# silvery107/rl-mpc-locomotion

Measured on AMD Instinct MI355X. Metric: MPC control steps/sec (whole node) @ horizon=10, 4096 robots; max |GRF| err vs OSQP, higher is better.
Workload: dtype f64; 1 GPU; config 2: 4096 robots/GPU x 1 GPU(s), Aliengo, trot, horizon=10, flat terrain (BASELINE configs[1]); one controller.run(dof_states, body_states, commands) -> torques call per step with EVERY robot due for its MPC update: state estimator, leg kinematics, gait / foot placement, compute_contact_forces (QP build + solve), swing / stance commands, leg-torque map a22 = SURVEY.md 8(d)'s unit of work; war; seam=ctrl, robots_per_gpu=4096, robots_total=4096, horizon=10, parallelism=robot-sharded x1

## Files before the change

rl-mpc-locomotion_amd/csrc/mpc_core.h:

```cpp
#pragma once

#include <math.h>
#include <stdint.h>

#if defined(__HIPCC__)
#define MPC_HD __host__ __device__ __forceinline__
#else
#define MPC_HD inline
#endif
#if defined(__HIP_DEVICE_COMPILE__)
#define MPC_LAUNDER(x) asm volatile("" : "+v"(x))
#define MPC_SCHED_FENCE() __builtin_amdgcn_sched_barrier(0)
#define MPC_LDS_STORE64(p, v) (*(volatile __attribute__((address_space(3))) double *)(p) = (v))
#define MPC_LDS_LOAD64(p) (*(const volatile __attribute__((address_space(3))) double *)(p))
typedef double mpc_double2 __attribute__((ext_vector_type(2)));
#define MPC_LDS_LOAD128(p, lo, hi) do { const mpc_double2 v2_ = *(const volatile __attribute__((address_space(3))) mpc_double2 *)(p); (lo) = v2_.x; (hi) = v2_.y; } while (0)
#define MPC_GST(p, v) __hip_atomic_store((p), (v), __ATOMIC_RELAXED, __HIP_MEMORY_SCOPE_AGENT)
#define MPC_GLD(p) __hip_atomic_load((p), __ATOMIC_RELAXED, __HIP_MEMORY_SCOPE_AGENT)
#define MPC_WAIT_LOADS() __builtin_amdgcn_s_waitcnt(0x0F70)
#define MPC_WAIT_LDS() __builtin_amdgcn_s_waitcnt(0xC07F)
#else
#define MPC_WAIT_LOADS() ((void)0)
#define MPC_WAIT_LDS() ((void)0)
#define MPC_GST(p, v) (*(p) = (v))
// ... 34 lines not shown
#define MPC_CLOCK() ((long long)__builtin_readcyclecounter())
#else
#define MPC_CLOCK() (0LL)
#endif

namespace mpc {

#if defined(__HIPCC__)
typedef _Float16 mpc_half;
MPC_HD double half_to_double(mpc_half v) { return (double)v; }
#else
typedef unsigned short mpc_half;
inline double half_to_double(mpc_half b) {
  const int sgn = b >> 15, ex = (b >> 10) & 31, man = b & 1023;
  double v;
  if (ex == 0) v = ldexp((double)man, -24);
  else if (ex == 31) v = man ? NAN : INFINITY;
  else v = ldexp((double)(man | 1024), ex - 25);
  return sgn ? -v : v;
}
#endif

constexpr double kRho0 = 0.1, kSigma = 1e-6, kAlphaRelax = 1.6;
constexpr double kEpsAbs = 1e-3, kEpsRel = 1e-3;
constexpr int kMaxIter = 4000, kCheck = 25;
constexpr double kRhoMin = 1e-6, kRhoMax = 1e6, kRhoEqOverIneq = 1e3, kRhoTol = 1e-4;
constexpr int kScalingIters = 10;
constexpr double kMinScaling = 1e-4, kMaxScaling = 1e4, kAdaptTol = 5.0;
constexpr double kInfty = 1e30, kDelta = 1e-6;
constexpr int kPolishRefine = 3;
constexpr double kGravity = 9.8, kMaxScale = 10.0, kMinScale = 0.1;

constexpr int kStSolved = 1, kStSolvedInaccurate = 2, kStPrimInfInaccurate = 3, kStDualInfInaccurate = 4, kStMaxIter = -2, kStPrimInf = -3, kStDualInf = -4,
              kStNonCvx = -7, kStUnsolved = -10;

constexpr int kAsPos[9] = {0, 2, 3, 5, 7, 8, 10, 11, 14};

template <int H>
struct Cfg {
  static constexpr int N = 12 * H, M = 20 * H, NF = 4 * H;
  static constexpr int TS = 6;
  static constexpr int G = N / TS;
  static constexpr int MT = G * (G + 1) / 2;
  static constexpr int NT = H > 16 ? MPC_NT_H20 : (H > 12 ? MPC_NT_H16 : 1);
  static constexpr int MTH = (MT + NT - 1) / NT;
  static constexpr int TE = TS * TS;
  static constexpr int T0 = (((MTH > N ? MTH : N) + 63) / 64) * 64;
  static constexpr int T = T0 < 128 ? 128 : T0;
  static constexpr int MR = (M + T - 1) / T;
  static constexpr int IN_LEN = 56 + 4 * H;
  static_assert(T <= 1024, "workgroup too large");
  static constexpr int NP = N + 2;
  static constexpr bool kQInLds = H > 12;
#ifdef MPC_PIN_MASK
  static constexpr int kPinMask = MPC_PIN_MASK;
#else
  static constexpr int kPinMask = H > 16 ? 3 : 17;
#endif
  static constexpr int QP_Q = 0, QP_BND = N, QP_CONE = N + 3 * NF, QP_B6 = QP_CONE + 16, QP_TH1 = QP_B6 + 72,
                       QP_TH2 = QP_TH1 + 36, QP_LEN = QP_TH2 + 8;
  static constexpr int SC_D = 0, SC_E = N, SC_QS = N + M, SC_C = 2 * N + M, SC_JOB = SC_C + 2, SC_LEN = SC_C + 4;
  static MPC_HD double scaled_cone_entry(const double *qp, const double *sc, int f, int k) {
    const int pos = kAsPos[k];
    return (qp[QP_CONE + pos] * sc[SC_E + 5 * f + pos / 3]) * sc[SC_D + 3 * f + pos % 3];
  }
  static MPC_HD double scaled_cone_entry(double a, double e, double d) { return (a * e) * d; }
  static constexpr int XQP_L = N, XQP_U = N + M, XQP_CONE = N + 2 * M, XQP_LEN = XQP_CONE + 16 + 72 + 36 + 8;
  static constexpr int XSC_AS = 2 * N + M, XSC_LS = XSC_AS + 15 * NF, XSC_US = XSC_LS + M, XSC_C = XSC_US + M, XSC_LEN = XSC_C + 4;
  static constexpr int NW = 6 * H, GW = H, MTW = H * (H + 1) / 2;
  static constexpr int FOOT0 = MPC_FOOT0(H, MTW);
  static constexpr int TWMIN = FOOT0 + NF > MTW ? FOOT0 + NF : MTW;
  static constexpr int TW = (((TWMIN > NW ? TWMIN : NW) + 63) / 64) * 64;
  static constexpr int NPW = NW + 2;
};

constexpr int IN_W = 0, IN_POS = 13, IN_VEL = 16, IN_RPY = 19, IN_NRM = 22, IN_ANG = 25, IN_CONTACT = 28;
template <int H> constexpr int in_foot() { return 28 + 4 * H; }
template <int H> constexpr int in_fric() { return 40 + 4 * H; }
template <int H> constexpr int in_dpos() { return 44 + 4 * H; }
template <int H> constexpr int in_dvel() { return 47 + 4 * H; }
template <int H> constexpr int in_drpy() { return 50 + 4 * H; }
template <int H> constexpr int in_dang() { return 53 + 4 * H; }

template <int H> constexpr int state_len() { return 2 * Cfg<H>::N + 2 * Cfg<H>::M + 2; }

constexpr int kInfoLen = 8;
constexpr int kProfLen = 16;

struct RobotModel {
  double mass, inv_mass, inv_inertia[9], dt, alpha;
};

#define MPC_V alignas(16) double
template <int H>
struct ScaleShared {
  using C = Cfg<H>;
  MPC_V q[C::kQInLds ? C::N : 2];
  MPC_V qs[C::N]; MPC_V As[C::NF * 15];
  MPC_V D[C::N]; MPC_V E[C::M];
  double c, cinv, ctmp;
  int first;
  MPC_V xt[C::N];
  MPC_V cone[16];
  MPC_V dt_[C::N]; MPC_V et_[C::M];
  MPC_V part[C::NP * C::G];
};
template <int H>
struct AsmShared {
  using C = Cfg<H>;
  MPC_V in[C::IN_LEN];
  static constexpr int XK = 13 * H > 74 ? 13 * H : 74;
  MPC_V x0[13]; MPC_V xref[13 * H]; MPC_V sdiff[XK]; MPC_V xk[XK];
  MPC_V a_dt[169]; MPC_V b_dt[156]; MPC_V a_exp[169]; MPC_V b_exp[156];
  MPC_V wanb[H * 156];
  MPC_V B6[72]; MPC_V th1[36]; MPC_V th2[8];
};
template <int H>
struct PrepShared {
  union {
    AsmShared<H> as;
    ScaleShared<H> sc;
  };
  MPC_V u12[288];
};
#undef MPC_V

template <int H>
struct Thread {
  using C = Cfg<H>;
  int tid;
  int ti[C::NT], tj[C::NT];
  bool mact[C::NT], dia[C::NT];
  double Mx[C::NT * C::TE];
  static constexpr int VPL = (C::N + 63) / 64;
  double rm[VPL];
  double red[2];
  MPC_HD void init(int id) {
    tid = id;
    for (int u = 0; u < C::NT; ++u) {
      const int tile = id + u * C::MTH;
      mact[u] = id < C::MTH && tile < C::MT;
      int r = 0;
      while ((r + 1) * (r + 2) / 2 <= tile) ++r;
      ti[u] = r; tj[u] = tile - r * (r + 1) / 2; dia[u] = ti[u] == tj[u];
    }
  }
};

struct TileView {
  int ti, tj, index;
  bool dia;
  double *Mx;
};

MPC_HD double limit_scaling(double v) {
  v = v < kMinScaling ? 1.0 : v;
  return v > kMaxScaling ? kMaxScaling : v;
}
MPC_HD double dmax(double a, double b) { return a > b ? a : b; }
MPC_HD double dmin(double a, double b) { return a < b ? a : b; }
MPC_HD double raw_max(double a, double b) {
#if defined(__HIP_DEVICE_COMPILE__)
  double r;
  asm("v_max_f64 %0, %1, %2" : "=v"(r) : "v"(a), "v"(b));
  return r;
#else
  return fmax(a, b);
#endif
}
MPC_HD double raw_min(double a, double b) {
#if defined(__HIP_DEVICE_COMPILE__)
  double r;
  asm("v_min_f64 %0, %1, %2" : "=v"(r) : "v"(a), "v"(b));
  return r;
#else
  return fmin(a, b);
#endif
}
MPC_HD double clampd(double v, double lo, double hi) { return raw_min(raw_max(v, lo), hi); }

MPC_HD int mpc_ffs64(unsigned long long v) {
#if defined(__HIP_DEVICE_COMPILE__)
  return __ffsll((long long)v) - 1;
#else
  return __builtin_ctzll(v);
#endif
}

MPC_HD unsigned long long dbits(double v) {
  union { double d; unsigned long long u; } c;
  c.d = v;
  return c.u;
}
MPC_HD double bitsd(unsigned long long u) {
  union { double d; unsigned long long u; } c;
  c.u = u;
  return c.d;
}

#ifndef MPC_PROFILE_SUB
#define MPC_PROFILE_SUB 0
#endif
#define MPC_SUBLAP(sec, k) do { if (MPC_PROFILE_SUB == (sec)) lap(k); } while (0)

template <int H, class Exec>
struct Assembler {
  using C = Cfg<H>;
  using Th = Thread<H>;
  static constexpr int N = C::N, M = C::M, NF = C::NF, T = C::T, TS = C::TS, TE = C::TE;

  Exec &ex;
  AsmShared<H> &s;
  const RobotModel &mdl;
  const float *in;
  const double *in64;
  const mpc_half *in16;
  double *u12;
  double *qp;
  long long *prof;
  long long tc[16] = {0, 0, 0, 0, 0, 0, 0, 0, 0, 0, 0, 0, 0, 0, 0, 0};
  long long tlast = 0;
#ifndef MPC_SECTION_PROFILE
  MPC_HD void lap(int) {}
#else
  MPC_HD void lap(int k) { const long long now = MPC_CLOCK(); tc[k] += now - tlast; tlast = now; }
#endif

  static MPC_HD double mat3e(const double *a, const double *b, int e) {
    const int i = e / 3, j = e - 3 * i;
    return a[3 * i] * b[j] + a[3 * i + 1] * b[3 + j] + a[3 * i + 2] * b[6 + j];
  }

  MPC_HD double in_at(int i) const { return in64 ? in64[i] : (in16 ? half_to_double(in16[i]) : (double)in[i]); }
  MPC_HD void run() {
    tlast = MPC_CLOCK();
    double *const trig = s.xk, *const fw = s.xk + 43, *const iw = s.xk + 64;
    double *const iib = s.sdiff + 53;
    static_assert(AsmShared<H>::XK >= 73, "xk / sdiff too small for the set-up scratch");
    ex.par([&](Th &t) {
      for (int i = t.tid; i < C::IN_LEN; i += T) s.in[i] = in_at(i);
      for (int i = t.tid; i < 169; i += T) s.a_dt[i] = 0;
      for (int i = t.tid; i < 156; i += T) s.b_dt[i] = 0;
      for (int i = t.tid; i < 72; i += T) { qp[C::QP_B6 + i] = 0; s.B6[i] = 0; }
      if (t.tid >= 64 && t.tid < 67) {
        const int k = t.tid - 64;
        const double ang = in_at(IN_RPY + k);
        trig[2 * k] = cos(ang); trig[2 * k + 1] = sin(ang);
        if (k == 1) trig[6] = tan(ang);
      } else if (t.tid >= 96 && t.tid < 105) {
        iib[t.tid - 96] = mdl.inv_inertia[t.tid - 96];
      }
    });
    MPC_SUBLAP(4, 9);
    ex.par([&](Th &t) {
      if (t.tid == 0) {
        const double cr = trig[0], sr = trig[1], cp = trig[2], sp = trig[3], cy = trig[4], sy = trig[5];
        const double rx[9] = {1.0, 0.0, 0.0, 0.0, cr, -sr, 0.0, sr, cr};
        const double ry[9] = {cp, 0.0, sp, 0.0, 1.0, 0.0, -sp, 0.0, cp};
        const double rz[9] = {cy, -sy, 0.0, sy, cy, 0.0, 0.0, 0.0, 1.0};
        double m1[9], m2[9], rxyz[9], rzyx[9], t2[9], ib[9];
#pragma unroll
        for (int e = 0; e < 9; ++e) { m1[e] = mat3e(rx, ry, e); m2[e] = mat3e(rz, ry, e); ib[e] = iib[e]; }
#pragma unroll
        for (int e = 0; e < 9; ++e) { rxyz[e] = mat3e(m1, rz, e); rzyx[e] = mat3e(m2, rx, e); }
        const double *fb = s.in + in_foot<H>();
#pragma unroll
        for (int i = 0; i < 4; ++i)
#pragma unroll
          for (int r = 0; r < 3; ++r) fw[3 * i + r] = rxyz[3 * r] * fb[3 * i] + rxyz[3 * r + 1] * fb[3 * i + 1] + rxyz[3 * r + 2] * fb[3 * i + 2];
#pragma unroll
        for (int e = 0; e < 9; ++e) t2[e] = mat3e(rzyx, ib, e);
#pragma unroll
        for (int i = 0; i < 3; ++i)
#pragma unroll
          for (int j = 0; j < 3; ++j) iw[3 * i + j] = t2[3 * i] * rzyx[3 * j] + t2[3 * i + 1] * rzyx[3 * j + 1] + t2[3 * i + 2] * rzyx[3 * j + 2];
      }
      if (t.tid >= 32 && t.tid < 45) {
        const int i = t.tid - 32;
        s.x0[i] = i < 3 ? s.in[IN_RPY + i] : i < 6 ? s.in[IN_POS + i - 3] : i < 9 ? s.in[IN_ANG + i - 6] : i < 12 ? s.in[IN_VEL + i - 9] : -kGravity;
      }
      for (int f = t.tid; f < NF; f += T) {
        const double cst = s.in[IN_CONTACT + f];
        const double fzmax = mdl.mass * kGravity * kMaxScale, fzmin = mdl.mass * kGravity * kMinScale;
        const double mu0 = s.in[in_fric<H>()];
        qp[C::QP_BND + 3 * f] = dmax(fzmin * cst, -kInfty);
        qp[C::QP_BND + 3 * f + 1] = dmin((mu0 + 1) * fzmax * cst, kInfty);
        qp[C::QP_BND + 3 * f + 2] = dmin(fzmax * cst, kInfty);
      }
      for (int k = t.tid; k < 13 * H; k += T) {
        const int i = k / 13, r = k - 13 * i;
        const double tt = mdl.dt * (i + 1);
        const int drpy = in_drpy<H>(), dvel = in_dvel<H>(), dang = in_dang<H>(), dpos = in_dpos<H>();
        const int bi = r < 2 ? drpy + r : r == 2 ? IN_RPY + 2 : r < 5 ? IN_POS + r - 3 : r == 5 ? dpos + 2 : r < 9 ? dang + r - 6 : dvel + (r < 11 ? r - 9 : 0);
        const int si = r == 2 ? dang + 2 : dvel + (r == 4 ? 1 : 0);
        const double base = s.in[bi], slope = s.in[si];
        const double v = (r == 2 || r == 3 || r == 4) ? tt * slope + base : base;
        s.xref[k] = r == 11 ? 0.0 : r == 12 ? -kGravity : v;
      }
    });
    MPC_SUBLAP(4, 12);
    ex.par([&](Th &t) {
      const double dt = mdl.dt;
      if (t.tid < 36) {
        const int i = t.tid / 9, e = t.tid - 9 * i, r = e / 3, c = e - 3 * r;
        const double *v = fw + 3 * i;
        double acc = 0;
        for (int k = 0; k < 3; ++k) {
          const double sk = (k == c) ? 0.0 : (((c - k + 3) % 3 == 1) ? -v[3 - k - c] : v[3 - k - c]);
          const double term = iw[3 * r + k] * sk;
          acc = k == 0 ? term : acc + term;
        }
        s.b_dt[(6 + r) * 12 + 3 * i + c] = acc * dt;
        qp[C::QP_B6 + r * 12 + 3 * i + c] = acc;
        s.B6[r * 12 + 3 * i + c] = acc;
      } else if (t.tid < 48) {
        const int k = t.tid - 36, i = k / 3, r = k - 3 * i;
        s.b_dt[(9 + r) * 12 + 3 * i + r] = mdl.inv_mass * dt;
        qp[C::QP_B6 + (3 + r) * 12 + 3 * i + r] = mdl.inv_mass;
        s.B6[(3 + r) * 12 + 3 * i + r] = mdl.inv_mass;
      } else if (t.tid < 57) {
        const int e = t.tid - 48, r = e / 3, c = e - 3 * r;
        const double cp = trig[2], cy = trig[4], sy = trig[5], tp = trig[6];
        const double num = c == 0 ? cy : sy;
        double val;
        if (c == 2) val = r == 2 ? 1.0 : 0.0;
        else if (r == 0) val = num / cp;
        else if (r == 1) val = c == 0 ? -sy : cy;
        else val = num * tp;
        s.a_dt[r * 13 + 6 + c] = val * dt;
      } else if (t.tid < 60) {
        const int r = t.tid - 57;
        s.a_dt[(3 + r) * 13 + 9 + r] = dt;
        s.a_dt[(9 + r) * 13 + 12] = s.in[IN_NRM + r] * dt;
      } else if (t.tid == 60) {
        const double *fr = s.in + in_fric<H>();
        const double cb[15] = {-1, 0, fr[0], 1, 0, fr[1], 0, -1, fr[2], 0, 1, fr[3], 0, 0, 1};
        for (int k = 0; k < 15; ++k) qp[C::QP_CONE + k] = cb[k];
      }
    });
    MPC_SUBLAP(1, 9);
    MPC_SUBLAP(4, 13);
    double *const U = s.a_exp;
    ex.par([&](Th &t) {
      for (int kk = t.tid; kk < 156; kk += T) {
        const int r = kk / 12, c = kk - 12 * r;
        double acc = 0;
        if (r < 3) { for (int j = 6; j < 9; ++j) acc += s.a_dt[r * 13 + j] * s.b_dt[j * 12 + c]; }
        else if (r < 6) acc += s.a_dt[r * 13 + r + 6] * s.b_dt[(r + 6) * 12 + c];
        s.b_exp[kk] = s.b_dt[kk] + acc / 2;
      }
      for (int e2 = T - 1 - t.tid; e2 < 72 + 13; e2 += T) {
        if (e2 < 72) {
          const int e = e2, r = e / 12, c = e - 12 * r;
          double acc = 0;
          if (r < 3) { for (int j = 6; j < 9; ++j) acc += s.a_dt[r * 13 + j] * s.b_dt[j * 12 + c]; }
          else acc = s.a_dt[r * 13 + r + 6] * s.b_dt[(r + 6) * 12 + c];
          U[e] = acc;
        } else {
          const int r = e2 - 72;
          double a1 = 0, a2 = 0;
          if (r < 3) { for (int j = 6; j < 9; ++j) a1 += s.a_dt[r * 13 + j] * s.x0[j]; }
          else if (r < 6) { a1 = s.a_dt[r * 13 + r + 6] * s.x0[r + 6]; a2 = (s.a_dt[r * 13 + r + 6] * s.a_dt[(r + 6) * 13 + 12]) * s.x0[12]; }
          else if (r >= 9 && r < 12) a1 = s.a_dt[r * 13 + 12] * s.x0[12];
          s.sdiff[r] = a1; s.sdiff[13 + r] = a2;
        }
      }
      if (t.tid < 36) {
        const int a = t.tid / 6, b = t.tid - 6 * a;
        const double dt = mdl.dt, d2 = 2.0 * dt * dt;
        double v = 0;
        if (a < 3 && b < 3) {
          for (int r = 0; r < 3; ++r) v += s.in[IN_W + r] * (s.a_dt[r * 13 + 6 + a] * s.a_dt[r * 13 + 6 + b]);
          v *= d2;
        } else if (a == b) v = (d2 * dt * dt) * s.in[IN_W + a];
        qp[C::QP_TH1 + t.tid] = v;
        s.th1[t.tid] = v;
      } else if (t.tid < 42) {
        const double v = (2.0 * mdl.dt * mdl.dt) * s.in[IN_W + 6 + t.tid - 36];
        qp[C::QP_TH2 + t.tid - 36] = v;
        s.th2[t.tid - 36] = v;
      }
    });
    MPC_SUBLAP(1, 10);
    ex.par([&](Th &t) {
      for (int e = t.tid; e < H * 156; e += T) {
        const int k = e / 156, rc = e - 156 * k, r = rc / 12;
        const double v = r < 6 ? s.b_exp[rc] + (double)k * U[rc] : s.b_exp[rc];
        s.wanb[e] = s.in[IN_W + r] * v;
      }
      for (int e = t.tid; e < 13 * (H - 1); e += T) {
        const int i = e / 13, r = e - 13 * i;
        const double kk = i + 1;
        s.xk[e] = s.x0[r] + kk * s.sdiff[r] + (kk * kk / 2) * s.sdiff[13 + r];
      }
    });
    MPC_SUBLAP(1, 11);
    ex.par([&](Th &t) {
      for (int k = t.tid; k < 13 * H; k += T) s.sdiff[k] = (k < 13 * (H - 1) ? s.xk[k] : 0.0) - s.xref[k];
    });
    lap(1);
    ex.par([&](Th &t) {
      for (int jc = t.tid; jc < N; jc += T) {
        const int j = jc / 12, c = jc - 12 * j;
        double acc = 0;
        for (int i = j; i < H; ++i) {
          const double *bk = s.wanb + (i - j) * 156 + c, *sd = s.sdiff + 13 * i;
          double e = 0, o = 0;
#pragma unroll
          for (int r = 0; r < 13; ++r) {
            if (r & 1) o += bk[r * 12] * sd[r];
            else e += bk[r * 12] * sd[r];
          }
          acc += e + o;
        }
        qp[C::QP_Q + jc] = 2 * acc;
      }
      for (int e = t.tid; e < 288; e += T) {
        const int which = e / 144, ab = e - 144 * which, a = ab / 12, b = ab - 12 * a;
        double acc = 0;
        if (which == 0) {
          for (int p = 0; p < 6; ++p) {
            double row = 0;
            for (int q = 0; q < 6; ++q) row += s.th1[6 * p + q] * s.B6[12 * q + b];
            acc += s.B6[12 * p + a] * row;
          }
        } else {
          for (int p = 0; p < 6; ++p) acc += s.B6[12 * p + a] * (s.th2[p] * s.B6[12 * p + b]);
        }
        u12[e] = acc;
      }
    });
    lap(2);
    if (prof) {
      ex.par([&](Th &t) {
        if (t.tid == 0) {
          prof[1] = tc[1]; prof[2] = tc[2];
          if (MPC_PROFILE_SUB == 1 || MPC_PROFILE_SUB == 4) for (int k = 9; k <= 13; ++k) prof[k] = tc[k];
        }
      });
    }
  }
};


template <int H, class Exec>
struct Scaler {
  using C = Cfg<H>;
  using Th = Thread<H>;
  using Sh = ScaleShared<H>;
  static constexpr int N = C::N, M = C::M, NF = C::NF, T = C::T, TS = C::TS, G = C::G, TE = C::TE, NP = C::NP;

  Exec &ex;
  Sh &s;
  const double *state;
  const double *u12;
  double alpha;
  const double *qp;
  double *sc;
  long long *prof = nullptr;
  long long tc[6] = {0, 0, 0, 0, 0, 0};
  long long tlast = 0;
  using Tv = TileView;
  template <class F>
  MPC_HD void for_tiles(Th &t, F &&f) {
#pragma unroll
    for (int u = 0; u < C::NT; ++u)
      if (t.mact[u]) {
        Tv v{t.ti[u], t.tj[u], t.tid + u * C::MTH, t.dia[u], t.Mx + u * TE};
        f(v, u);
      }
  }
  template <class F>
  MPC_HD void for_rows(const Th &t, F &&f) {
#pragma unroll
    for (int p = 0; p < C::MR; ++p) {
      const int i = t.tid + p * T;
      if (i < M) f(i);
    }
  }
  MPC_HD void pin_tiles(int site) {
#if defined(__HIP_DEVICE_COMPILE__)
    if (!((C::kPinMask >> site) & 1)) return;
#pragma unroll
    for (int e = 0; e < C::NT * TE; ++e) MPC_LAUNDER(ex.th.Mx[e]);
#endif
  }
  MPC_HD double q_at(int i) const {
    if constexpr (C::kQInLds) return s.q[i];
    else return qp[C::QP_Q + i];
  }
#ifndef MPC_SECTION_PROFILE
  MPC_HD void lap(int) {}
#else
  MPC_HD void lap(int k) { const long long now = MPC_CLOCK(); tc[k] += now - tlast; tlast = now; }
#endif
  template <bool MAX>
  static MPC_HD double fold_parts(const Sh &s, int row) {
    double v[G];
#pragma unroll
    for (int k = 0; k < G; ++k) v[k] = MPC_LDS_LOAD64(s.part + k * NP + row);
#pragma unroll
    for (int w = 1; w < G; w *= 2)
#pragma unroll
      for (int k = 0; k + w < G; k += 2 * w) v[k] = MAX ? raw_max(v[k], v[k + w]) : v[k] + v[k + w];
    return v[0];
  }
  static MPC_HD double max_parts(const Sh &s, int row) { return fold_parts<true>(s, row); }
  MPC_HD void tile_rownorms(const Tv &t, const double *D) {
    double dc[TS], dr[TS], mr[TS], mc[TS];
#pragma unroll
    for (int b = 0; b < TS; ++b) { dc[b] = D ? D[TS * t.tj + b] : 1.0; dr[b] = D ? D[TS * t.ti + b] : 1.0; mr[b] = 0; mc[b] = 0; }
#pragma unroll
    for (int a = 0; a < TS; ++a)
#pragma unroll
      for (int b = 0; b < TS; ++b) {
        const double m = fabs(t.Mx[a * TS + b]);
        mr[a] = fmax(mr[a], m * dc[b]);
        mc[b] = fmax(mc[b], m * dr[a]);
      }
    double *pd = s.part + t.tj * NP + TS * t.ti, *pt = s.part + t.ti * NP + TS * t.tj;
#pragma unroll
    for (int a = 0; a < TS; ++a) pd[a] = mr[a] * dr[a];
    if (!t.dia) {
#pragma unroll
      for (int b = 0; b < TS; ++b) pt[b] = mc[b] * dc[b];
    }
  }
  MPC_HD void build_tile(Tv &t) {
    const int sr = t.ti >> 1, sc_ = t.tj >> 1, rh = t.ti & 1, ch = t.tj & 1;
    const double m = (double)(H - sr), d = (double)(sr - sc_);
    const double s2 = m * (4.0 * m * m - 1.0) / 12.0 + d * (m * m) * 0.5;
    const double *u1 = u12 + (6 * rh) * 12 + 6 * ch, *u2 = u1 + 144;
#pragma unroll
    for (int a = 0; a < TS; ++a)
#pragma unroll
      for (int b = 0; b < TS; ++b) {
        double v = s2 * u1[12 * a + b] + m * u2[12 * a + b];
        if (t.dia && a == b) v += alpha;
        t.Mx[a * TS + b] = v;
      }
  }
  static MPC_HD double fast_rsqrt(double d) {
// ... 18 lines not shown
#endif
  }
  template <bool COST, bool DUPD>
  MPC_HD void fold_phase() {
    ex.seq([&](Th &t) {
      if (t.tid < 64) {
        double sum = 0, qm = 0;
#pragma unroll
        for (int v = 0; v < Th::VPL; ++v) {
          const int j = t.tid + 64 * v;
          if (j < N) {
            const double m = max_parts(s, j);
            t.rm[v] = m;
            if constexpr (COST) { sum += m; qm = raw_max(qm, fabs(s.qs[j])); }
          }
        }
        t.red[0] = sum; t.red[1] = qm;
      }
    });
    if constexpr (COST) ex.wave_sum_max([](Th &t) { return t.red; });
    ex.par([&](Th &t) {
      if (t.tid < 64) {
        double ct = 1.0;
        if constexpr (COST) {
          const double mean = (s.c * t.red[0]) * (1.0 / N);
          ct = fast_recip(limit_scaling(fmax(mean, limit_scaling(t.red[1]))));
        }
#pragma unroll
        for (int v = 0; v < Th::VPL; ++v) {
          const int j = t.tid + 64 * v;
          if (j < N) {
            if constexpr (DUPD) {
              const int f = j / 3, c = j - 3 * f;
              double mx = (s.c * ct) * t.rm[v];
#pragma unroll
              for (int r = 0; r < 5; ++r) mx = fmax(mx, fabs(s.As[15 * f + 3 * r + c]));
              const double d = fast_rsqrt(limit_scaling(mx));
              s.dt_[j] = d;
              s.D[j] *= d;
            } else {
              s.qs[j] *= ct;
            }
          }
        }
        if (t.tid == 0) s.ctmp = DUPD ? ct : s.c * ct;
      }
    });
  }
  static MPC_HD double row_scale3(double a0, double a1, double a2) {
    return fast_rsqrt(limit_scaling(fmax(fmax(fabs(a0), fabs(a1)), fabs(a2))));
  }
  MPC_HD void scale() {
    tlast = MPC_CLOCK();
    ex.par([&](Th &t) {
      for_tiles(t, [&](Tv &v, int) { build_tile(v); tile_rownorms(v, nullptr); });
      if (t.tid < N) {
        s.qs[t.tid] = s.first ? q_at(t.tid) : s.xt[t.tid];
        s.D[t.tid] = 1.0;
      }
      for_rows(t, [&](int i) {
        const double *a = s.cone + 3 * (i % 5);
        s.E[i] = 1.0;
        s.et_[i] = row_scale3(a[0], a[1], a[2]);
      });
      for (int k = t.tid; k < NF * 15; k += T) s.As[k] = s.cone[k % 15];
      if (t.tid == 0) s.c = 1.0;
    });
    lap(3);
    pin_tiles(5);
    fold_phase<false, true>();
    for (int it = 0; it < kScalingIters; ++it) {
      pin_tiles(7);
      ex.par([&](Th &t) {
        const double ct = s.ctmp;
        for_tiles(t, [&](Tv &v, int) { tile_rownorms(v, s.D); });
        for_rows(t, [&](int i) {
          const int f = i / 5;
          double *a = s.As + 3 * i;
          const double e = s.et_[i], a0 = a[0], a1 = a[1], a2 = a[2];
          const double d0 = s.dt_[3 * f], d1 = s.dt_[3 * f + 1], d2 = s.dt_[3 * f + 2], eo = s.E[i];
          const double n0 = (a0 * e) * d0, n1 = (a1 * e) * d1, n2 = (a2 * e) * d2;
          a[0] = n0; a[1] = n1; a[2] = n2;
          s.E[i] = eo * e;
          s.et_[i] = row_scale3(n0, n1, n2);
        });
        if (t.tid < N) s.qs[t.tid] = (s.qs[t.tid] * ct) * s.dt_[t.tid];
        if (t.tid == T - 1) s.c *= ct;
      });
      if (it + 1 < kScalingIters) fold_phase<true, true>();
      else fold_phase<true, false>();
    }
    lap(4);
    pin_tiles(6);
    ex.par([&](Th &t) {
      const double cf = s.ctmp;
      if (t.tid == 0) { sc[C::SC_C] = cf; sc[C::SC_C + 1] = 1.0 / cf; }
      if (t.tid < N) {
        const double qv = s.first ? s.qs[t.tid] : (s.D[t.tid] * q_at(t.tid)) * cf;
        sc[C::SC_QS + t.tid] = qv;
        sc[C::SC_D + t.tid] = s.D[t.tid];
      }
      for_rows(t, [&](int i) { sc[C::SC_E + i] = s.E[i]; });
    });
    lap(5);
    if (prof) {
      ex.par([&](Th &t) { if (t.tid == 0) { prof[3] = tc[3]; prof[4] = tc[4]; prof[5] = tc[5]; } });
    }
  }

  MPC_HD void load() {
    ex.par([&](Th &t) {
      for (int i = t.tid; i < N; i += T) { if constexpr (C::kQInLds) s.q[i] = qp[C::QP_Q + i]; s.xt[i] = state[N + 2 * M + i];  }
      if (t.tid < 15) s.cone[t.tid] = qp[C::QP_CONE + t.tid];
      if (t.tid == 0) s.first = state[2 * N + 2 * M + 1] == 0.0;
    });
  }
  MPC_HD void run() {
    load();
    scale();
  }
};

}
```

rl-mpc-locomotion_amd/csrc/mpc_device.h:

```cpp
#pragma once
#include <hip/hip_runtime.h>

namespace mpc {

constexpr int kWaitVm0 = 0x0F70;

template <int CTRL>
__device__ __forceinline__ double quad_perm(double v) {
  int lo = __double2loint(v), hi = __double2hiint(v);
  lo = __builtin_amdgcn_mov_dpp(lo, CTRL, 0xF, 0xF, true);
  hi = __builtin_amdgcn_mov_dpp(hi, CTRL, 0xF, 0xF, true);
  return __hiloint2double(hi, lo);
}
constexpr int quad_ctrl(int a, int b, int c, int d) { return a | (b << 2) | (c << 4) | (d << 6); }
__device__ __forceinline__ double read_lane(double v, int lane) {
  const int lo = __builtin_amdgcn_readlane(__double2loint(v), lane), hi = __builtin_amdgcn_readlane(__double2hiint(v), lane);
  return __hiloint2double(hi, lo);
}

template <class TH, bool WAVE = false>
struct DeviceExec {
  TH &th;
  __device__ __forceinline__ TH &first() { return th; }
  template <class F>
  __device__ __forceinline__ void par(F &&f) {
    f(th);
    if constexpr (WAVE) {
      __builtin_amdgcn_fence(__ATOMIC_ACQ_REL, "wavefront");
      __builtin_amdgcn_wave_barrier();
    } else __syncthreads();
  }
  template <class F>
  __device__ __forceinline__ void seq(F &&f) { f(th); }
  template <int N, class A>
  __device__ __forceinline__ void quad_allsum(A &&acc) {
    double *v = acc(th);
#pragma unroll
    for (int i = 0; i < N; ++i) {
      const double a = v[i] + quad_perm<quad_ctrl(1, 0, 3, 2)>(v[i]);
      v[i] = a + quad_perm<quad_ctrl(2, 3, 0, 1)>(a);
    }
  }
  template <class S, class D>
  __device__ __forceinline__ void quad_scatter6(S &&src, D &&dst) {
    const double *w = src(th);
    double *g = dst(th);
    const bool odd = threadIdx.x & 1, hi = threadIdx.x & 2;
    double a[3];
#pragma unroll
    for (int p = 0; p < 3; ++p) {
      const double keep = odd ? w[2 * p + 1] : w[2 * p], give = odd ? w[2 * p] : w[2 * p + 1];
      a[p] = keep + quad_perm<quad_ctrl(1, 0, 3, 2)>(give);
    }
    const double keep = hi ? a[1] : a[0], give = hi ? a[0] : a[1];
    g[0] = keep + quad_perm<quad_ctrl(2, 3, 0, 1)>(give);
    g[1] = a[2] + quad_perm<quad_ctrl(2, 3, 0, 1)>(a[2]);
  }
  template <class A>
  __device__ __forceinline__ void wave_sum_max(A &&acc) {
    double *v = acc(th);
    double a = v[0], m = v[1];
    a += quad_perm<quad_ctrl(1, 0, 3, 2)>(a);  m = fmax(m, quad_perm<quad_ctrl(1, 0, 3, 2)>(m));
    a += quad_perm<quad_ctrl(2, 3, 0, 1)>(a);  m = fmax(m, quad_perm<quad_ctrl(2, 3, 0, 1)>(m));
    a += quad_perm<0x141>(a);                  m = fmax(m, quad_perm<0x141>(m));
    a += quad_perm<0x140>(a);                  m = fmax(m, quad_perm<0x140>(m));
    v[0] = (read_lane(a, 0) + read_lane(a, 16)) + (read_lane(a, 32) + read_lane(a, 48));
    v[1] = fmax(fmax(read_lane(m, 0), read_lane(m, 16)), fmax(read_lane(m, 32), read_lane(m, 48)));
  }
  template <class V, class I>
  __device__ __forceinline__ void wg_argmax(V &&val, I &&idx, double *scratch) {
    double *v = val(th);
    if constexpr (WAVE) {
      double m = v[0];
      m = fmax(m, quad_perm<quad_ctrl(1, 0, 3, 2)>(m));
      m = fmax(m, quad_perm<quad_ctrl(2, 3, 0, 1)>(m));
      m = fmax(m, quad_perm<0x141>(m));
      m = fmax(m, quad_perm<0x140>(m));
      m = fmax(fmax(read_lane(m, 0), read_lane(m, 16)), fmax(read_lane(m, 32), read_lane(m, 48)));
      const unsigned long long who = __ballot(v[0] == m);
      idx(th) = who ? __ffsll((long long)who) - 1 : 0;
      v[0] = m;
    } else {
      double m = v[0];
// ... 58 lines not shown
```

rl-mpc-locomotion_amd/csrc/mpc_horizon.hip:

```cpp
#include <hip/hip_runtime.h>

#ifndef MPC_H
#error "compile with -DMPC_H=<planning horizon>"
#endif
#define MPC_LOCKSTEP 1
#include "mpc_horizon.h"
#include "mpc_device.h"
#include "mpc_wrench.h"
#include "mpc_exact32.h"

using namespace mpc;

#ifndef MPC_SCALE_MIN_WAVES
#define MPC_SCALE_MIN_WAVES 3
#endif
#ifndef MPC_MIN_WAVES_MAX_T
#define MPC_MIN_WAVES_MAX_T 256
#endif
#ifndef MPC_SOLVE_MIN_WAVES
#define MPC_SOLVE_MIN_WAVES 1
#endif
#ifndef MPC_SOLVE_MIN_WAVES_WIDE
#define MPC_SOLVE_MIN_WAVES_WIDE 2
#endif
// ... 139 lines not shown
    int bk[kPer], rank[kPer];
#pragma unroll
    for (int i = 0; i < kPer; ++i) {
      const int r = r0 + i * blockDim.x + threadIdx.x;
      bk[i] = -1;
      if (r < n && (!active || active[r])) {
        const long long c = prof[(size_t)r * kProfLen + kProfLen - 1] >> 14;
        unsigned char *hr = hist + (size_t)r * kOrderHistory;
        hr[slot] = (unsigned char)(c < 0 ? 0 : (c >= kOrderBuckets ? kOrderBuckets - 1 : c));
        int mx = 0;
#pragma unroll
        for (int k = 0; k < kOrderHistory; ++k) mx = max(mx, (int)hr[k]);
        bk[i] = mx;
        rank[i] = atomicAdd(&cnt[bk[i]], 1);
      }
    }
    __syncthreads();
    if (threadIdx.x == 0) {
      int acc = filled;
      for (int b = kOrderBuckets - 1; b >= 0; --b) { base[b] = acc; acc += cnt[b]; cnt[b] = 0; }
      filled = acc;
    }
    __syncthreads();
#pragma unroll
    for (int i = 0; i < kPer; ++i)
      if (bk[i] >= 0) order[base[bk[i]] + rank[i]] = r0 + i * blockDim.x + threadIdx.x;
    __syncthreads();
  }
  if (threadIdx.x == 0) { sched[kSchedNext] = 0; sched[kSchedHead] = 0; sched[kSchedTail] = 0; sched[kSchedJobs] = filled; }
}

template <int H>
__global__ __launch_bounds__(Cfg<H>::T, (Cfg<H>::T <= MPC_MIN_WAVES_MAX_T && Cfg<H>::NT == 1 ? MPC_SCALE_MIN_WAVES : 1)) void mpc_prep_kernel(
    int n, const RobotModel *__restrict__ models, const float *__restrict__ in, const double *__restrict__ in64, const _Float16 *__restrict__ in16, const double *__restrict__ state,
    double *__restrict__ qp, double *__restrict__ sc, long long *__restrict__ prof, const int *__restrict__ active, int *__restrict__ order,
    unsigned char *__restrict__ hist, int hist_slot, int *__restrict__ sched, int *__restrict__ ready) {
  __shared__ __attribute__((aligned(16))) PrepShared<H> sh;
  using C = Cfg<H>;
  if (blockIdx.x == 0) {
    order_block(n, prof, hist, hist_slot, order, active, sched, ready);
    return;
  }
  const int robot = (int)blockIdx.x - 1;
  if (robot >= n) return;
  if (active && !active[robot]) return;
  Thread<H> th;
  th.init(threadIdx.x);
#pragma unroll
  for (int j = 0; j < C::NT * C::TE; ++j) th.Mx[j] = 0;
  using Ex = DeviceExec<Thread<H>>;
  Ex ex{th};
  const RobotModel &mdl = models[robot];
  double *qpr = qp + (size_t)robot * C::QP_LEN;
  Assembler<H, Ex> am{ex, sh.as, mdl, in ? in + (size_t)robot * C::IN_LEN : nullptr, in64 ? in64 + (size_t)robot * C::IN_LEN : nullptr, in16 ? in16 + (size_t)robot * C::IN_LEN : nullptr, sh.u12, qpr, prof ? prof + (size_t)robot * kProfLen : nullptr};
  am.run();
  Scaler<H, Ex> sk{ex, sh.sc, state + (size_t)robot * state_len<H>(), sh.u12, mdl.alpha, qpr, sc + (size_t)robot * C::SC_LEN, prof ? prof + (size_t)robot * kProfLen : nullptr};
  sk.run();
}

template <int H>
int launch(const LaunchArgs &a) {
  if (a.ev) (void)hipEventRecord(a.ev[0], a.stream);
  hipLaunchKernelGGL(mpc_prep_kernel<H>, dim3(a.n + 1), dim3(Cfg<H>::T), 0, a.stream, a.n, a.models, a.in, a.in64, a.in16, a.state, a.qp, a.sc, a.prof, a.active, a.order, a.hist,
                     a.hist_slot, a.sched, a.ready);
  if (a.ev) (void)hipEventRecord(a.ev[1], a.stream);
  if (a.exact) {
    if (a.f32_seed && a.seed) hipLaunchKernelGGL((mpc_exact32_kernel<H>), dim3(a.n), dim3(64), 0, a.stream, a.models, a.qp, a.sc, a.order, a.sched, a.seed);
    hipLaunchKernelGGL((mpc_exact_kernel<H>), dim3(a.n), dim3(Cfg<H>::TW), 0, a.stream, a.models, a.state, a.qp, a.sc, a.forces, a.info, a.prof, a.order, a.sched, a.ready, a.seed);
    hipLaunchKernelGGL((mpc_solve_kernel<H, true>), dim3(a.n), dim3(Cfg<H>::TW), 0, a.stream, a.n, a.models, a.state, a.qp, a.sc, a.forces, a.info, a.prof, a.order, a.sched, a.ready,
                       a.max_iter);
  }
  else if (a.job_slots > 0) {
    int slots = Cfg<H>::TW <= 64 ? a.job_slots : a.job_slots / 2;
    if (slots < 1) slots = 1;
    hipLaunchKernelGGL((mpc_solve_jobs_kernel<H>), dim3(a.n < slots ? a.n : slots), dim3(Cfg<H>::TW), 0, a.stream, a.models, a.state, a.qp, a.sc, a.forces, a.info, a.prof, a.order,
                       a.sched, a.ready, a.max_iter);
  }
  else hipLaunchKernelGGL((mpc_solve_kernel<H, false>), dim3(a.n), dim3(Cfg<H>::TW), 0, a.stream, a.n, a.models, a.state, a.qp, a.sc, a.forces, a.info, a.prof, a.order, a.sched,
                          a.ready, a.max_iter);
  if (a.ev) (void)hipEventRecord(a.ev[2], a.stream);
  return (int)hipGetLastError();
}

template <int H>
void expand_records(const double *qp, const double *sc, double *xqp, double *xsc) {
  using C = Cfg<H>;
  if (xqp) {
    for (int i = 0; i < C::N; ++i) xqp[i] = qp[C::QP_Q + i];
    for (int f = 0; f < C::NF; ++f)
      for (int r = 0; r < 5; ++r) {
        xqp[C::XQP_L + 5 * f + r] = r < 4 ? 0.0 : qp[C::QP_BND + 3 * f];
        xqp[C::XQP_U + 5 * f + r] = r < 4 ? qp[C::QP_BND + 3 * f + 1] : qp[C::QP_BND + 3 * f + 2];
      }
    for (int i = 0; i < 16 + 72 + 36 + 8; ++i) xqp[C::XQP_CONE + i] = qp[C::QP_CONE + i];
  }
  if (xsc) {
    for (int i = 0; i < 2 * C::N + C::M; ++i) xsc[i] = sc[i];
    for (int f = 0; f < C::NF; ++f) {
      for (int k = 0; k < 15; ++k) xsc[C::XSC_AS + 15 * f + k] = 0.0;
      for (int k = 0; k < 9; ++k) xsc[C::XSC_AS + 15 * f + kAsPos[k]] = C::scaled_cone_entry(qp, sc, f, k);
      for (int r = 0; r < 5; ++r) {
        const double e = sc[C::SC_E + 5 * f + r];
        xsc[C::XSC_LS + 5 * f + r] = e * (r < 4 ? 0.0 : qp[C::QP_BND + 3 * f]);
        xsc[C::XSC_US + 5 * f + r] = e * (r < 4 ? qp[C::QP_BND + 3 * f + 1] : qp[C::QP_BND + 3 * f + 2]);
      }
    }
    for (int i = 0; i < 4; ++i) xsc[C::XSC_C + i] = sc[C::SC_C + i];
  }
}
// ... 10 lines not shown
```

Before: 2.600 million control steps/s.

## Cut barriers in QP prep kernel with wave-local phases and register handoffs

Restructures the per-robot prep kernel (QP assembly and scaling) to use fewer workgroup barriers. The single-thread rotation/inertia phase now runs wave-local, while other waves fill A/B/cone entries in the same phase. The q vector, the warm-start state and the first-iteration flag are kept in registers and prefetched at kernel start rather than in a separate load pass. Two small phases are merged, and the q and u12 loops are split across disjoint thread groups. The risk is subtle ordering bugs in wave_par, which only fences at wavefront scope while other waves read trig/fw afterwards through later barriers.

```diff
diff --git a/rl-mpc-locomotion_amd/csrc/mpc_core.h b/rl-mpc-locomotion_amd/csrc/mpc_core.h
--- a/rl-mpc-locomotion_amd/csrc/mpc_core.h
+++ b/rl-mpc-locomotion_amd/csrc/mpc_core.h
@@ -110,6 +110,8 @@
   static_assert(T <= 1024, "workgroup too large");
   static constexpr int NP = N + 2;
   static constexpr bool kQInLds = H > 12;
+  static constexpr int QT = ((N + 63) / 64) * 64;
+  static constexpr bool kSplitQU = (T - QT) * 3 >= 288;
 #ifdef MPC_PIN_MASK
   static constexpr int kPinMask = MPC_PIN_MASK;
 #else
@@ -157,9 +159,6 @@
   MPC_V qs[C::N]; MPC_V As[C::NF * 15];
   MPC_V D[C::N]; MPC_V E[C::M];
   double c, cinv, ctmp;
-  int first;
-  MPC_V xt[C::N];
-  MPC_V cone[16];
   MPC_V dt_[C::N]; MPC_V et_[C::M];
   MPC_V part[C::NP * C::G];
 };
@@ -179,7 +178,7 @@
     AsmShared<H> as;
     ScaleShared<H> sc;
   };
-  MPC_V u12[288];
+  MPC_V u12[288 + 16];
 };
 #undef MPC_V
 
@@ -193,6 +192,8 @@
   static constexpr int VPL = (C::N + 63) / 64;
   double rm[VPL];
   double red[2];
+  double qreg, qold;
+  bool first;
   MPC_HD void init(int id) {
     tid = id;
     for (int u = 0; u < C::NT; ++u) {
@@ -290,27 +291,46 @@
   }
 
   MPC_HD double in_at(int i) const { return in64 ? in64[i] : (in16 ? half_to_double(in16[i]) : (double)in[i]); }
+  MPC_HD void in_at2(int i, int j, double &a, double &b) const {
+    if (in64) { a = in64[i]; b = in64[j]; }
+    else if (in16) { const mpc_half x = in16[i], y = in16[j]; a = half_to_double(x); b = half_to_double(y); }
+    else { const float x = in[i], y = in[j]; a = (double)x; b = (double)y; }
+  }
+  template <class E, class F>
+  static MPC_HD auto wave_phase(E &e, F &&f, int) -> decltype(e.wave_par(f)) { return e.wave_par(f); }
+  template <class E, class F>
+  static MPC_HD void wave_phase(E &e, F &&f, long) { e.par(f); }
+  template <class F>
+  MPC_HD void wpar(F &&f) { wave_phase(ex, f, 0); }
+
   MPC_HD void run() {
     tlast = MPC_CLOCK();
     double *const trig = s.xk, *const fw = s.xk + 43, *const iw = s.xk + 64;
     double *const iib = s.sdiff + 53;
     static_assert(AsmShared<H>::XK >= 73, "xk / sdiff too small for the set-up scratch");
+    static_assert(C::IN_LEN <= T && N <= T && T >= 128, "one input entry and one variable per thread, a wavefront beside the first");
+    constexpr int W = T / 64;
+    constexpr int kCosWave = 1, kSinWave = W > 2 ? 2 : 1, kTanWave = W > 3 ? 3 : W - 1;
     ex.par([&](Th &t) {
-      for (int i = t.tid; i < C::IN_LEN; i += T) s.in[i] = in_at(i);
+      const int lane = t.tid & 63, ka = lane < 3 ? lane : 0;
+      const double ii = mdl.inv_inertia[t.tid >= T - 9 ? t.tid - (T - 9) : 0];
+      double iv, ang;
+      in_at2(t.tid < C::IN_LEN ? t.tid : 0, IN_RPY + ka, iv, ang);
+      MPC_WAIT_LOADS();
+      if (t.tid < C::IN_LEN) s.in[t.tid] = iv;
+      if (t.tid >= T - 9) iib[t.tid - (T - 9)] = ii;
       for (int i = t.tid; i < 169; i += T) s.a_dt[i] = 0;
       for (int i = t.tid; i < 156; i += T) s.b_dt[i] = 0;
       for (int i = t.tid; i < 72; i += T) { qp[C::QP_B6 + i] = 0; s.B6[i] = 0; }
-      if (t.tid >= 64 && t.tid < 67) {
-        const int k = t.tid - 64;
-        const double ang = in_at(IN_RPY + k);
-        trig[2 * k] = cos(ang); trig[2 * k + 1] = sin(ang);
-        if (k == 1) trig[6] = tan(ang);
-      } else if (t.tid >= 96 && t.tid < 105) {
-        iib[t.tid - 96] = mdl.inv_inertia[t.tid - 96];
+      if (lane < 3) {
+        const int w = t.tid >> 6;
+        if (w == kCosWave) trig[2 * lane] = cos(ang);
+        if (w == kSinWave) trig[2 * lane + 1] = sin(ang);
+        if (w == kTanWave && lane == 1) trig[6] = tan(ang);
       }
     });
     MPC_SUBLAP(4, 9);
-    ex.par([&](Th &t) {
+    wpar([&](Th &t) {
       if (t.tid == 0) {
         const double cr = trig[0], sr = trig[1], cp = trig[2], sp = trig[3], cy = trig[4], sy = trig[5];
         const double rx[9] = {1.0, 0.0, 0.0, 0.0, cr, -sr, 0.0, sr, cr};
@@ -333,11 +353,42 @@
 #pragma unroll
           for (int j = 0; j < 3; ++j) iw[3 * i + j] = t2[3 * i] * rzyx[3 * j] + t2[3 * i + 1] * rzyx[3 * j + 1] + t2[3 * i + 2] * rzyx[3 * j + 2];
       }
-      if (t.tid >= 32 && t.tid < 45) {
-        const int i = t.tid - 32;
-        s.x0[i] = i < 3 ? s.in[IN_RPY + i] : i < 6 ? s.in[IN_POS + i - 3] : i < 9 ? s.in[IN_ANG + i - 6] : i < 12 ? s.in[IN_VEL + i - 9] : -kGravity;
-      }
-      for (int f = t.tid; f < NF; f += T) {
+    });
+    auto x0_at = [&](int i) { return i < 3 ? s.in[IN_RPY + i] : i < 6 ? s.in[IN_POS + i - 3] : i < 9 ? s.in[IN_ANG + i - 6] : i < 12 ? s.in[IN_VEL + i - 9] : -kGravity; };
+    auto rest = [&](Th &t) {
+      constexpr int TO = T - 64;
+      constexpr int bA = TO >= 128 ? 64 : 16, bM = TO >= 192 ? 128 : 32;
+      const int o = t.tid - 64;
+      if (o < 0) return;
+      const double dt = mdl.dt;
+      if (o < 13) s.x0[o] = x0_at(o);
+      if (o >= bA && o < bA + 9) {
+        const int e = o - bA, r = e / 3, c = e - 3 * r;
+        const double cp = trig[2], cy = trig[4], sy = trig[5], tp = trig[6];
+        const double num = c == 0 ? cy : sy;
+        double val;
+        if (c == 2) val = r == 2 ? 1.0 : 0.0;
+        else if (r == 0) val = num / cp;
+        else if (r == 1) val = c == 0 ? -sy : cy;
+        else val = num * tp;
+        s.a_dt[r * 13 + 6 + c] = val * dt;
+      }
+      if (o >= bM && o < bM + 12) {
+        const int k = o - bM, i = k / 3, r = k - 3 * i;
+        s.b_dt[(9 + r) * 12 + 3 * i + r] = mdl.inv_mass * dt;
+        qp[C::QP_B6 + (3 + r) * 12 + 3 * i + r] = mdl.inv_mass;
+        s.B6[(3 + r) * 12 + 3 * i + r] = mdl.inv_mass;
+      } else if (o >= bM + 12 && o < bM + 15) {
+        const int r = o - (bM + 12);
+        s.a_dt[(3 + r) * 13 + 9 + r] = dt;
+        s.a_dt[(9 + r) * 13 + 12] = s.in[IN_NRM + r] * dt;
+      } else if (o >= bM + 16 && o < bM + 31) {
+        const int k = o - (bM + 16), r = k / 3, c = k - 3 * r;
+        const double v = c == 2 ? (r < 4 ? s.in[in_fric<H>() + (r < 4 ? r : 0)] : 1.0) : (r == 2 * c ? -1.0 : r == 2 * c + 1 ? 1.0 : 0.0);
+        qp[C::QP_CONE + k] = v;
+        u12[288 + k] = v;
+      }
+      for (int f = o; f < NF; f += TO) {
         const double cst = s.in[IN_CONTACT + f];
         const double fzmax = mdl.mass * kGravity * kMaxScale, fzmin = mdl.mass * kGravity * kMinScale;
         const double mu0 = s.in[in_fric<H>()];
@@ -345,7 +396,7 @@
         qp[C::QP_BND + 3 * f + 1] = dmin((mu0 + 1) * fzmax * cst, kInfty);
         qp[C::QP_BND + 3 * f + 2] = dmin(fzmax * cst, kInfty);
       }
-      for (int k = t.tid; k < 13 * H; k += T) {
+      for (int k = o; k < 13 * H; k += TO) {
         const int i = k / 13, r = k - 13 * i;
         const double tt = mdl.dt * (i + 1);
         const int drpy = in_drpy<H>(), dvel = in_dvel<H>(), dang = in_dang<H>(), dpos = in_dpos<H>();
@@ -355,9 +406,9 @@
         const double v = (r == 2 || r == 3 || r == 4) ? tt * slope + base : base;
         s.xref[k] = r == 11 ? 0.0 : r == 12 ? -kGravity : v;
       }
-    });
+    };
     MPC_SUBLAP(4, 12);
-    ex.par([&](Th &t) {
+    wpar([&](Th &t) {
       const double dt = mdl.dt;
       if (t.tid < 36) {
         const int i = t.tid / 9, e = t.tid - 9 * i, r = e / 3, c = e - 3 * r;
@@ -371,34 +422,13 @@
         s.b_dt[(6 + r) * 12 + 3 * i + c] = acc * dt;
         qp[C::QP_B6 + r * 12 + 3 * i + c] = acc;
         s.B6[r * 12 + 3 * i + c] = acc;
-      } else if (t.tid < 48) {
-        const int k = t.tid - 36, i = k / 3, r = k - 3 * i;
-        s.b_dt[(9 + r) * 12 + 3 * i + r] = mdl.inv_mass * dt;
-        qp[C::QP_B6 + (3 + r) * 12 + 3 * i + r] = mdl.inv_mass;
-        s.B6[(3 + r) * 12 + 3 * i + r] = mdl.inv_mass;
-      } else if (t.tid < 57) {
-        const int e = t.tid - 48, r = e / 3, c = e - 3 * r;
-        const double cp = trig[2], cy = trig[4], sy = trig[5], tp = trig[6];
-        const double num = c == 0 ? cy : sy;
-        double val;
-        if (c == 2) val = r == 2 ? 1.0 : 0.0;
-        else if (r == 0) val = num / cp;
-        else if (r == 1) val = c == 0 ? -sy : cy;
-        else val = num * tp;
-        s.a_dt[r * 13 + 6 + c] = val * dt;
-      } else if (t.tid < 60) {
-        const int r = t.tid - 57;
-        s.a_dt[(3 + r) * 13 + 9 + r] = dt;
-        s.a_dt[(9 + r) * 13 + 12] = s.in[IN_NRM + r] * dt;
-      } else if (t.tid == 60) {
-        const double *fr = s.in + in_fric<H>();
-        const double cb[15] = {-1, 0, fr[0], 1, 0, fr[1], 0, -1, fr[2], 0, 1, fr[3], 0, 0, 1};
-        for (int k = 0; k < 15; ++k) qp[C::QP_CONE + k] = cb[k];
-      }
-    });
+      }
+    });
+    ex.par(rest);
     MPC_SUBLAP(1, 9);
     MPC_SUBLAP(4, 13);
     double *const U = s.a_exp;
+    double *const ax1 = s.xk, *const ax2 = s.xk + 13;
     ex.par([&](Th &t) {
       for (int kk = t.tid; kk < 156; kk += T) {
         const int r = kk / 12, c = kk - 12 * r;
@@ -417,10 +447,10 @@
         } else {
           const int r = e2 - 72;
           double a1 = 0, a2 = 0;
-          if (r < 3) { for (int j = 6; j < 9; ++j) a1 += s.a_dt[r * 13 + j] * s.x0[j]; }
-          else if (r < 6) { a1 = s.a_dt[r * 13 + r + 6] * s.x0[r + 6]; a2 = (s.a_dt[r * 13 + r + 6] * s.a_dt[(r + 6) * 13 + 12]) * s.x0[12]; }
-          else if (r >= 9 && r < 12) a1 = s.a_dt[r * 13 + 12] * s.x0[12];
-          s.sdiff[r] = a1; s.sdiff[13 + r] = a2;
+          if (r < 3) { for (int j = 6; j < 9; ++j) a1 += s.a_dt[r * 13 + j] * s.in[IN_ANG + j - 6]; }
+          else if (r < 6) { a1 = s.a_dt[r * 13 + r + 6] * s.in[IN_VEL + r - 3]; a2 = (s.a_dt[r * 13 + r + 6] * s.a_dt[(r + 6) * 13 + 12]) * -kGravity; }
+          else if (r >= 9 && r < 12) a1 = s.a_dt[r * 13 + 12] * -kGravity;
+          ax1[r] = a1; ax2[r] = a2;
         }
       }
       if (t.tid < 36) {
@@ -446,20 +476,19 @@
         const double v = r < 6 ? s.b_exp[rc] + (double)k * U[rc] : s.b_exp[rc];
         s.wanb[e] = s.in[IN_W + r] * v;
       }
-      for (int e = t.tid; e < 13 * (H - 1); e += T) {
-        const int i = e / 13, r = e - 13 * i;
+      for (int k = t.tid; k < 13 * H; k += T) {
+        const int i = k / 13, r = k - 13 * i;
         const double kk = i + 1;
-        s.xk[e] = s.x0[r] + kk * s.sdiff[r] + (kk * kk / 2) * s.sdiff[13 + r];
+        double xk = 0.0;
+        if (k < 13 * (H - 1)) xk = s.x0[r] + kk * ax1[r] + (kk * kk / 2) * ax2[r];
+        s.sdiff[k] = xk - s.xref[k];
       }
     });
     MPC_SUBLAP(1, 11);
-    ex.par([&](Th &t) {
-      for (int k = t.tid; k < 13 * H; k += T) s.sdiff[k] = (k < 13 * (H - 1) ? s.xk[k] : 0.0) - s.xref[k];
-    });
     lap(1);
     ex.par([&](Th &t) {
-      for (int jc = t.tid; jc < N; jc += T) {
-        const int j = jc / 12, c = jc - 12 * j;
+      if (t.tid < N) {
+        const int jc = t.tid, j = jc / 12, c = jc - 12 * j;
         double acc = 0;
         for (int i = j; i < H; ++i) {
           const double *bk = s.wanb + (i - j) * 156 + c, *sd = s.sdiff + 13 * i;
@@ -471,9 +500,11 @@
           }
           acc += e + o;
         }
-        qp[C::QP_Q + jc] = 2 * acc;
-      }
-      for (int e = t.tid; e < 288; e += T) {
+        t.qreg = 2 * acc;
+        qp[C::QP_Q + jc] = t.qreg;
+      }
+      for (int e = C::kSplitQU ? t.tid - C::QT : t.tid; e < 288; e += C::kSplitQU ? T - C::QT : T) {
+        if (e < 0) break;
         const int which = e / 144, ab = e - 144 * which, a = ab / 12, b = ab - 12 * a;
         double acc = 0;
         if (which == 0) {
@@ -490,7 +521,7 @@
     });
     lap(2);
     if (prof) {
-      ex.par([&](Th &t) {
+      ex.seq([&](Th &t) {
         if (t.tid == 0) {
           prof[1] = tc[1]; prof[2] = tc[2];
           if (MPC_PROFILE_SUB == 1 || MPC_PROFILE_SUB == 4) for (int k = 9; k <= 13; ++k) prof[k] = tc[k];
@@ -518,6 +549,7 @@
   long long *prof = nullptr;
   long long tc[6] = {0, 0, 0, 0, 0, 0};
   long long tlast = 0;
+  bool prefetched = false;
   using Tv = TileView;
   template <class F>
   MPC_HD void for_tiles(Th &t, F &&f) {
@@ -543,9 +575,9 @@
     for (int e = 0; e < C::NT * TE; ++e) MPC_LAUNDER(ex.th.Mx[e]);
 #endif
   }
-  MPC_HD double q_at(int i) const {
-    if constexpr (C::kQInLds) return s.q[i];
-    else return qp[C::QP_Q + i];
+  MPC_HD double q_own(const Th &t) const {
+    if constexpr (C::kQInLds) return s.q[t.tid];
+    else return t.qreg;
   }
 #ifndef MPC_SECTION_PROFILE
   MPC_HD void lap(int) {}
@@ -670,18 +702,24 @@
   }
   MPC_HD void scale() {
     tlast = MPC_CLOCK();
+    const double *const cone = u12 + 288;
     ex.par([&](Th &t) {
+      if (!prefetched) {
+        if (t.tid < N) t.qold = state[N + 2 * M + t.tid];
+        t.first = state[2 * N + 2 * M + 1] == 0.0;
+      }
       for_tiles(t, [&](Tv &v, int) { build_tile(v); tile_rownorms(v, nullptr); });
       if (t.tid < N) {
-        s.qs[t.tid] = s.first ? q_at(t.tid) : s.xt[t.tid];
+        if constexpr (C::kQInLds) s.q[t.tid] = t.qreg;
+        s.qs[t.tid] = t.first ? t.qreg : t.qold;
         s.D[t.tid] = 1.0;
       }
       for_rows(t, [&](int i) {
-        const double *a = s.cone + 3 * (i % 5);
+        const double *a = cone + 3 * (i % 5);
         s.E[i] = 1.0;
         s.et_[i] = row_scale3(a[0], a[1], a[2]);
       });
-      for (int k = t.tid; k < NF * 15; k += T) s.As[k] = s.cone[k % 15];
+      for (int k = t.tid; k < NF * 15; k += T) s.As[k] = cone[k % 15];
       if (t.tid == 0) s.c = 1.0;
     });
     lap(3);
@@ -714,7 +752,7 @@
       const double cf = s.ctmp;
       if (t.tid == 0) { sc[C::SC_C] = cf; sc[C::SC_C + 1] = 1.0 / cf; }
       if (t.tid < N) {
-        const double qv = s.first ? s.qs[t.tid] : (s.D[t.tid] * q_at(t.tid)) * cf;
+        const double qv = t.first ? s.qs[t.tid] : (s.D[t.tid] * q_own(t)) * cf;
         sc[C::SC_QS + t.tid] = qv;
         sc[C::SC_D + t.tid] = s.D[t.tid];
       }
@@ -722,21 +760,11 @@
     });
     lap(5);
     if (prof) {
-      ex.par([&](Th &t) { if (t.tid == 0) { prof[3] = tc[3]; prof[4] = tc[4]; prof[5] = tc[5]; } });
+      ex.seq([&](Th &t) { if (t.tid == 0) { prof[3] = tc[3]; prof[4] = tc[4]; prof[5] = tc[5]; } });
     }
   }
 
-  MPC_HD void load() {
-    ex.par([&](Th &t) {
-      for (int i = t.tid; i < N; i += T) { if constexpr (C::kQInLds) s.q[i] = qp[C::QP_Q + i]; s.xt[i] = state[N + 2 * M + i];  }
-      if (t.tid < 15) s.cone[t.tid] = qp[C::QP_CONE + t.tid];
-      if (t.tid == 0) s.first = state[2 * N + 2 * M + 1] == 0.0;
-    });
-  }
-  MPC_HD void run() {
-    load();
-    scale();
-  }
+  MPC_HD void run() { scale(); }
 };
 
 }
diff --git a/rl-mpc-locomotion_amd/csrc/mpc_device.h b/rl-mpc-locomotion_amd/csrc/mpc_device.h
--- a/rl-mpc-locomotion_amd/csrc/mpc_device.h
+++ b/rl-mpc-locomotion_amd/csrc/mpc_device.h
@@ -29,6 +29,12 @@
       __builtin_amdgcn_fence(__ATOMIC_ACQ_REL, "wavefront");
       __builtin_amdgcn_wave_barrier();
     } else __syncthreads();
+  }
+  template <class F>
+  __device__ __forceinline__ void wave_par(F &&f) {
+    if (__builtin_amdgcn_readfirstlane((int)threadIdx.x) < 64) f(th);
+    __builtin_amdgcn_fence(__ATOMIC_ACQ_REL, "wavefront");
+    __builtin_amdgcn_wave_barrier();
   }
   template <class F>
   __device__ __forceinline__ void seq(F &&f) { f(th); }
diff --git a/rl-mpc-locomotion_amd/csrc/mpc_horizon.hip b/rl-mpc-locomotion_amd/csrc/mpc_horizon.hip
--- a/rl-mpc-locomotion_amd/csrc/mpc_horizon.hip
+++ b/rl-mpc-locomotion_amd/csrc/mpc_horizon.hip
@@ -215,9 +215,13 @@
   Ex ex{th};
   const RobotModel &mdl = models[robot];
   double *qpr = qp + (size_t)robot * C::QP_LEN;
+  const double *st = state + (size_t)robot * state_len<H>();
+  th.qold = st[C::N + 2 * C::M + ((int)threadIdx.x < C::N ? (int)threadIdx.x : 0)];
+  th.first = st[2 * C::N + 2 * C::M + 1] == 0.0;
   Assembler<H, Ex> am{ex, sh.as, mdl, in ? in + (size_t)robot * C::IN_LEN : nullptr, in64 ? in64 + (size_t)robot * C::IN_LEN : nullptr, in16 ? in16 + (size_t)robot * C::IN_LEN : nullptr, sh.u12, qpr, prof ? prof + (size_t)robot * kProfLen : nullptr};
   am.run();
-  Scaler<H, Ex> sk{ex, sh.sc, state + (size_t)robot * state_len<H>(), sh.u12, mdl.alpha, qpr, sc + (size_t)robot * C::SC_LEN, prof ? prof + (size_t)robot * kProfLen : nullptr};
+  Scaler<H, Ex> sk{ex, sh.sc, st, sh.u12, mdl.alpha, qpr, sc + (size_t)robot * C::SC_LEN, prof ? prof + (size_t)robot * kProfLen : nullptr};
+  sk.prefetched = true;
   sk.run();
 }
 
```

New measurement: 2.637 million control steps/s (median of 6 runs). 1.4% higher.
